# MarvelMathesh/sincformer-metacog-speech-enhancement

Measured on AMD Instinct MI355X. Metric: audio frames/sec/GPU (16 kHz, 512-frame utts) + mask RMSE vs CPU ref, higher is better.
Workload: dtype fp16 MFMA operands (PerceptionAgent, fusion, Conformer GEMMs, heads) + bf16 attention core, fp32 accumulate (ops.POLICIES['mixed']); 1 GPU; B256 x 512-frame utterances (L40880, T512) forward; batch_per_gpu=256, samples=40880, frames_per_utt=512, launch=eager launches, streams=3, precision_policy=mixed

## Files before the change

include/sincformer_hip.h:

```cpp
#ifndef SINCFORMER_HIP_H
#define SINCFORMER_HIP_H
#ifdef __cplusplus
extern "C" {
#endif

#define SFM_OK 0
#define SFM_ERR_ARG (-1)
#define SFM_ERR_SHAPE (-2)
#define SFM_ERR_LAUNCH (-3)
#define SFM_DT_BF16 0
#define SFM_DT_F16 1

#define SFM_EPI_NONE 0
#define SFM_EPI_SWISH 1
#define SFM_EPI_GELU 2
#define SFM_EPI_RESID 3
#define SFM_EPI_GLU 4
#define SFM_EPI_SIGMOID 5
#define SFM_EPI_TANH_SCALE 6
#define SFM_EPI_SIGMA 7
#define SFM_EPI_CPEA 8

int sfm_abi_version(void);

// ... 195 lines not shown
int sfm_layernorm_bwd_ex(const float* x, const float* gamma, const void* dy, int dy_16, const float* dres, float* dx,
                         float* dgamma, float* dbeta, int M, int D, int ldx, int ldy, int ld, float eps, int dtype,
                         float* ws, void* stream);
int sfm_layernorm_bwd_next(const float* x, const float* gamma, const void* dy, int dy_16, const float* dres, float* dx,
                           float* dgamma, float* dbeta, int M, int D, int ldx, int ldy, int ld, float eps, int dtype,
                           void* next16, float next_alpha, float next_p, unsigned int next_seed, float* ws, void* stream);
int sfm_ew_train(const void* z, const void* g, void* out, long long M, int N, int mode, int g_f32, int out_f32,
                 float alpha, float p, unsigned int seed, int dtype, void* stream);
long long sfm_col_stats_ws_floats(int M, int C);
int sfm_col_stats(const float* y, const float* aux, const float* mean, const float* rstd, float* S, int M, int C, float* ws,
                  void* stream);
int sfm_add_cols(const float* a, const float* b, float* out, long long M, int C, int Cb, long long lda, long long ldb, long long ldo,
                 void* stream);
int sfm_lstm_hprev16(const float* h, void* out, int B, int T, int H, int dtype, void* stream);
int sfm_bn_finalize(const float* S, const float* gamma, const float* beta, float* run_mean, float* run_var, float* mean,
                    float* rstd, float* sc, float* sh, int C, long long M, float eps, float momentum, int eval_mode,
                    void* stream);
int sfm_bn_swish_bwd(const void* g, const float* y, const float* mean, const float* rstd, const float* gamma,
                     const float* beta, float* S, float* dy, int M, int C, int g_f32, int pass, int dtype,
                     float* ws, void* stream);
long long sfm_dwconv_wgrad_scratch_floats(int B, int T, int C, int KS);
int sfm_dwconv_wgrad(const void* x, const float* dy, float* dw, float* db, float* scratch, int B, int T, int C, int KS,
                     int dtype, void* stream);
int sfm_attention_fwd_train(const void* qkv, void* out, float* lse, int B, int T, int H, int hd, int ldqkv,
                            int ldo, int koff, int voff, long long qkv_batch_stride, long long o_batch_stride,
                            float scale, float p_drop, unsigned int seed, int dtype, void* stream);
int sfm_attention_bwd(const void* qkv, const void* O, const void* dO, const float* lse, float* delta, void* dqkv,
                      int B, int T, int H, int hd, int ldqkv, int ldo, int koff, int voff, float p_drop,
                      unsigned int seed, int dtype, void* stream);
int sfm_lin256(const void* A, const void* W, const float* bias, void* out, int M, int NW, int lda, int ldo, int glu, int dtype,
               int out_dtype, void* stream);
int sfm_ln_lin256(const float* X32, int ldx, const float* lnw, const float* lnb, float eps, const void* W, const float* bias,
                  void* out, int M, int NW, int ldo, int glu, int dtype, int out_dtype, void* stream);
int sfm_headpool_frames_per_tile(int Tin, int Tout);
int sfm_headpool(const void* xd, const void* W, const float* bias, void* pooled, float* gn_partial, int B, int Tin, int Tout, int NW,
                 int lda, int ldp, int gcols, int dtype, void* stream);

int sfm_bilstm_layer(const float* xg, const float* whh, float* out, int B, int T, int H, int dtype, void* stream);
int sfm_bilstm_layer_ex(const float* xg, const float* whh, float* out, int B, int T, int H, int w16, void* stream);
int sfm_bilstm_layer_train_ex(const float* xg, const float* whh, float* out, float* save, int B, int T, int H, int w16, void* stream);
int sfm_bilstm_layer_train(const float* xg, const float* whh, float* out, float* save, int B, int T, int H, int dtype,
                           void* stream);
int sfm_bilstm_layer_bwd(const float* save, const float* whh, const float* dout, float* dxg, int B, int T, int H,
                         void* stream);
int sfm_memory_fwd(const float* emb, const float* params, float* bias_out, float* gate_out, int* top_idx,
                   float* sim_out, int B, int key_dim, int value_dim, int slots, float temperature, void* stream);
long long sfm_memory_param_floats(int key_dim, int value_dim, int slots);
int sfm_memory_bwd(const float* emb, const float* params, const float* d_out, const float* d_gate, float* d_emb,
                   float* dparams, int B, int key_dim, int value_dim, int slots, float temperature, float* ws, void* stream);

int sfm_pstoi_loss(const float* e0, const float* e1, const float* c0, const float* c1, const float* band_w, float* loss,
                   float* g0, float* g1, double* ws, int B, int T, int F, int NB, int frame_len, float beta_db, int layout,
                   void* stream);
int sfm_mse_loss(const float* pred, const float* target, float* loss, float* grad, double* ws, long long n, void* stream);

#ifdef __cplusplus
}
#endif
#endif
```

sincformer_metacog_speech_enhancement_amd/csrc/pointwise.hip:

```cpp
#include "sfm_common.h"

template <class T>
__global__ __launch_bounds__(256) void layernorm_kernel(const float* __restrict__ x, const float* __restrict__ w,
                                                        const float* __restrict__ bsh, u16* out16, float* out32,
                                                        int M, int D, int ldx, int ld16, int ld32, float eps, int act) {
  const int lane = threadIdx.x & 63;
  const int row = blockIdx.x * 4 + (threadIdx.x >> 6);
  if (row >= M) return;
  const float* xr = x + (long long)row * ldx;
  float v[8];
  float s = 0.f;
#pragma unroll
  for (int i = 0; i < 8; ++i) {
    int d = lane + 64 * i;
    v[i] = (d < D) ? xr[d] : 0.f;
    s += v[i];
  }
  const float mean = wave_sum(s) / (float)D;
  float q = 0.f;
#pragma unroll
  for (int i = 0; i < 8; ++i) {
    int d = lane + 64 * i;
    float c = (d < D) ? (v[i] - mean) : 0.f;
    q += c * c;
  }
  const float rstd = rsqrtf(wave_sum(q) / (float)D + eps);
#pragma unroll
  for (int i = 0; i < 8; ++i) {
    int d = lane + 64 * i;
    if (d < D) {
      float y = (v[i] - mean) * rstd * w[d] + bsh[d];
      if (act == 1) y = gelu_erf(y);
      if (out16) out16[(long long)row * ld16 + d] = T::from_f32(y);
// ... 993 lines not shown
  const long long total = M * F;
  for (long long e = (long long)blockIdx.x * 256 + threadIdx.x; e < total; e += (long long)gridDim.x * 256) {
    const long long m = e / F;
    const int f = (int)(e - m * F);
    const float r = re[e], i = im[e];
    const float gr = g[m * ld_g + f], gi = g[m * ld_g + F + f];
    const float mag = sqrtf(r * r + i * i + 1e-8f);
    const float nf = log1pf(mag) / mag;
    const float c = (gr * r + gi * i) * (1.0f / (1.0f + mag) - nf) / (mag * mag);
    dre[e] = gr * nf + c * r;
    dim_[e] = gi * nf + c * i;
  }
}

extern "C" int sfm_stft_lognorm_bwd(const float* re, const float* im, const float* g, float* dre, float* dim_, long long M, int F,
                                    long long ld_g, void* stream) {
  if (!re || !im || !g || !dre || !dim_) return SFM_ERR_ARG;
  if (M <= 0 || F <= 0 || ld_g < 2 * F) return SFM_ERR_SHAPE;
  long long nb = (M * F + 255) / 256;
  if (nb > 16384) nb = 16384;
  SFM_LAUNCH(stft_lognorm_bwd_kernel, dim3((unsigned)nb), dim3(256), 0, (hipStream_t)stream, re, im, g, dre, dim_, M, F, ld_g);
  return SFM_OK;
}

__global__ __launch_bounds__(256) void polar_mask_kernel(const float* __restrict__ lm, const float* __restrict__ lp,
                                                         const float* __restrict__ mag_bias, const float* __restrict__ nr,
                                                         const float* __restrict__ ni, float* mr, float* mi, float* er,
                                                         float* ei, float* mmag, long long rows_per_batch, int F,
                                                         long long total, float phase_scale, long long ld_l,
                                                         long long ld_enh) {
  for (long long e = (long long)blockIdx.x * 256 + threadIdx.x; e < total; e += (long long)gridDim.x * 256) {
    long long m = e / F;
    int f = (int)(e - m * F);
    float a = lm[m * ld_l + f];
    if (mag_bias) a += mag_bias[(m / rows_per_batch) * F + f];
    float mg = 1.0f / (1.0f + expf(-a));
    float ph = tanhf(lp[m * ld_l + f]) * phase_scale;
    float c = cosf(ph), s = sinf(ph);
    float xr = mg * c, xi = mg * s;
    if (mr) mr[e] = xr;
    if (mi) mi[e] = xi;
    if (mmag) mmag[e] = mg;
    if (er) {
      float r = nr[e], i = ni[e];
      er[m * ld_enh + f] = xr * r - xi * i;
      ei[m * ld_enh + f] = xr * i + xi * r;
    }
  }
}

extern "C" int sfm_polar_mask(const float* lm, const float* lp, const float* mag_bias, const float* nr, const float* ni,
                              float* mr, float* mi, float* er, float* ei, float* mmag, int B, long long rows_per_batch,
                              int F, float phase_scale, long long ld_logits, long long ld_enh, void* stream) {
  if (!lm || !lp) return SFM_ERR_ARG;
  if (er && (!ei || !nr || !ni)) return SFM_ERR_ARG;
  long long total = (long long)B * rows_per_batch * F;
  if (total <= 0) return SFM_ERR_SHAPE;
  long long nb = (total + 255) / 256;
  if (nb > 16384) nb = 16384;
  SFM_LAUNCH(polar_mask_kernel, dim3((unsigned)nb), dim3(256), 0, (hipStream_t)stream, lm, lp, mag_bias, nr, ni,
                     mr, mi, er, ei, mmag, rows_per_batch, F, total, phase_scale, ld_logits, ld_enh);
  return SFM_OK;
}

__global__ __launch_bounds__(256) void complex_mul_kernel(const float* __restrict__ sr, const float* __restrict__ si,
                                                          const float* __restrict__ mr, const float* __restrict__ mi,
                                                          float* er, float* ei, long long total) {
  for (long long e = (long long)blockIdx.x * 256 + threadIdx.x; e < total; e += (long long)gridDim.x * 256) {
    float a = sr[e], b = si[e], c = mr[e], d = mi[e];
    er[e] = c * a - d * b;
    ei[e] = c * b + d * a;
  }
}

extern "C" int sfm_complex_mul(const float* sr, const float* si, const float* mr, const float* mi, float* er, float* ei,
                               long long total, void* stream) {
  if (!sr || !si || !mr || !mi || !er || !ei) return SFM_ERR_ARG;
  if (total <= 0) return SFM_ERR_SHAPE;
  long long nb = (total + 255) / 256;
// ... 145 lines not shown
```

sincformer_metacog_speech_enhancement_amd/functional.py:

```python
import math
import numpy as np
import torch

from . import ops

N_FFT, HOP, WIN = 256, 80, 160
N_FREQ = N_FFT // 2 + 1
SINC_ON_16BIT_MFMA = True
FUSE_LD = 1088


def _f32(t):
    return t.detach().float().contiguous()


def sub(sd, prefix):
    p = prefix + "."
    return {k[len(p):]: v for k, v in sd.items() if k.startswith(p)}


def add_to16(x32, y32, C):
    M = x32.numel() // C
    dev = x32.device
    one = _const(dev, C, 1.0)
# ... 350 lines not shown
    with ops.stage("block", pk.get("index")):
        return _block_forward(x32, pk, B, T, H, want16, seg)


def _block_forward(x32, pk, B, T, H, want16, seg=None):
    if _ffn_fusable(x32, pk["ff1"]) and x32.shape[1] == 256:
        x, h = ffn_forward_ln(x32, pk["ff1"], pk["mhsa"]["ln_w"], pk["mhsa"]["ln_b"], False, True)
        x = mhsa_forward(x, pk["mhsa"], B, T, H, h=h, index=pk.get("index"), seg=seg)
        x = convmod_forward(x, pk["conv"], B, T, seg=seg)
        if not want16 and _ffn_fusable(x, pk["ff2"]):
            return ffn_forward_ln(x, pk["ff2"], pk["fn_w"], pk["fn_b"], True, False)[1]
        x = ffn_forward(x, pk["ff2"])
    else:
        x = ffn_forward(x32, pk["ff1"])
        x = mhsa_forward(x, pk["mhsa"], B, T, H, index=pk.get("index"), seg=seg)
        x = convmod_forward(x, pk["conv"], B, T, seg=seg)
        x = ffn_forward(x, pk["ff2"])
    out = torch.empty_like(x)
    out16 = torch.empty(x.shape, device=x.device, dtype=ops.compute_dtype()) if want16 else None
    ops.layernorm(x, pk["fn_w"], pk["fn_b"], out16=out16, out32=out)
    return (out, out16) if want16 else out


def pack_complex_conformer(sd, num_blocks, num_heads=4):
    nf2 = sd["input_proj.weight"].shape[1]
    with ops.stage("front"):
        win = ops.pack_linear(sd["input_proj.weight"], sd["input_proj.bias"], k_pad_to=ops.round_up(nf2, 64))
    with ops.stage("tail"):
        wout = ops.pack_linear(sd["output_proj.weight"], sd["output_proj.bias"])
    return {"in": win, "out": wout,
            "blocks": [pack_block(sub(sd, "blocks.%d" % i), num_heads, i) for i in range(num_blocks)], "nf2": nf2}


def complex_conformer_core(x16, pk, B, T, H, out_dtype=None):
    with ops.stage("front"):
        x = ops.linear16(x16, pk["in"], out_dtype=torch.float32)
    skip = x
    for bp in pk["blocks"]:
        x = block_forward(x, bp, B, T, H)
    with ops.stage("tail"):
        y16 = add_to16(x, skip, x.shape[1])
        return ops.linear16(y16, pk["out"], out_dtype=out_dtype or ops.compute_dtype())


def complex_conformer_forward(stft_real, stft_imag, pk, H):
    B, T, nf = stft_real.shape
    M = B * T
    sr, si = stft_real.contiguous(), stft_imag.contiguous()
    ld = pk["in"].Kpad
    with ops.stage("front"):
        x16 = torch.empty(M, ld, device=sr.device, dtype=ops.compute_dtype())
        ops.convert_rows(sr, x16, M, nf, nf, nf, ld)
        ops.convert_rows(si, x16[:, nf:], M, nf, ld - nf, nf, ld)
    y = complex_conformer_core(x16, pk, B, T, H, out_dtype=torch.float32).reshape(B, T, 2 * nf)
    return y[..., :nf], y[..., nf:]


def pack_perception(sd, sample_rate):
    with ops.stage("pa"):
        return _pack_perception(sd, sample_rate)


def _pack_perception(sd, sample_rate):
    pk = {"fs": float(sample_rate)}
    for k in ("low_hz_", "band_hz_", "window", "n_"):
        pk[k] = _f32(sd["sinc_conv." + k]).reshape(-1)
    pk["K"] = pk["window"].numel()
    pk["C0"] = pk["low_hz_"].numel()
    pk["sn_w"], pk["sn_b"] = _f32(sd["sinc_norm.weight"]), _f32(sd["sinc_norm.bias"])
    pk["blocks"] = []
    for i in range(3):
        s = sub(sd, "conv_blocks.%d" % i)
# ... 187 lines not shown
        h = ops.bilstm_layer(xg, lp["whh"], B, T, H, w16=ops.lstm_w16())
        x16 = torch.empty(M, 2 * H, device=h.device, dtype=dt)
        ops.convert_rows(h, x16, M, 2 * H, 2 * H, 2 * H, 2 * H)
    oc = pk["oc"]
    if out is None:
        out = torch.empty(M, 4 * oc, device=x16.device, dtype=torch.float32)
    ops.linear16(x16, pk["heads"], epi=ops.EPI_CPEA, alpha=math.pi, nsplit=2 * oc, out=out)
    return out


def pack_memory_params(sd):
    order = ["key_proj.0.weight", "key_proj.0.bias", "key_proj.1.weight", "key_proj.1.bias", "key_proj.3.weight",
             "key_proj.3.bias", "keys", "values", "value_proj.0.weight", "value_proj.0.bias", "gate.0.weight",
             "gate.0.bias"]
    return torch.cat([_f32(sd[k]).reshape(-1) for k in order]).contiguous()


def pack_msa(sd, num_blocks, num_heads=4):
    with ops.stage("front"):
        pk = {"f0": ops.pack_linear(sd["fusion.0.weight"], sd["fusion.0.bias"], k_pad_to=FUSE_LD),
              "f1w": _f32(sd["fusion.1.weight"]), "f1b": _f32(sd["fusion.1.bias"]),
              "f3": ops.pack_linear(sd["fusion.3.weight"], sd["fusion.3.bias"]),
              "f4w": _f32(sd["fusion.4.weight"]), "f4b": _f32(sd["fusion.4.bias"])}
    pk["conf"] = pack_complex_conformer(sub(sd, "conformer"), num_blocks, num_heads)
    with ops.stage("tail"):
        pk.update({"r0": ops.pack_linear(sd["mask_proj_real.0.weight"], sd["mask_proj_real.0.bias"]),
                   "r2": ops.pack_linear(sd["mask_proj_real.2.weight"], sd["mask_proj_real.2.bias"]),
                   "i0": ops.pack_linear(sd["mask_proj_imag.0.weight"], sd["mask_proj_imag.0.bias"]),
                   "i2": ops.pack_linear(sd["mask_proj_imag.2.weight"], sd["mask_proj_imag.2.bias"])})
    pk["d_model"] = sd["fusion.3.weight"].shape[0]
    return pk


def msa_logits(fused16, pk, B, T, H):
    D = pk["d_model"]
    with ops.stage("front"):
        h = ops.linear16(fused16, pk["f0"], out_dtype=torch.float32)
        h16 = _ln16(h, pk["f1w"], pk["f1b"], act=1)
        h = ops.linear16(h16, pk["f3"], out_dtype=torch.float32)
        hf16 = _ln16(h, pk["f4w"], pk["f4b"])
    y16 = complex_conformer_core(hf16, pk["conf"], B, T, H)
    half = D // 2
    with ops.stage("tail"):
        gr = ops.linear16(y16[:, :half], pk["r0"], epi=ops.EPI_GELU)
        lm = ops.linear16(gr, pk["r2"], out_dtype=torch.float32)
        gi = ops.linear16(y16[:, half:], pk["i0"], epi=ops.EPI_GELU)
        lp = ops.linear16(gi, pk["i2"], out_dtype=torch.float32)
    return lm, lp


def msa_pack_inputs(z_real, z_imag, cpea, noisy_real, noisy_imag):
    with ops.stage("front"):
        return _msa_pack_inputs(z_real, z_imag, cpea, noisy_real, noisy_imag)


def _msa_pack_inputs(z_real, z_imag, cpea, noisy_real, noisy_imag):
    B, D, T = z_real.shape
    M = B * T
    dev = z_real.device
    fused = torch.empty(M, FUSE_LD, device=dev, dtype=ops.compute_dtype())
    zr, zi = z_real.float().contiguous(), z_imag.float().contiguous()
    ops.transpose(zr, fused, B, D, T, D * T, T, T * FUSE_LD, FUSE_LD)
    ops.transpose(zi, fused[:, D:], B, D, T, D * T, T, T * FUSE_LD, FUSE_LD)
    col = 2 * D
    for k in ("rho_s", "rho_n", "phi1", "phi2"):
        c = cpea[k].float().contiguous()
        oc = c.shape[-1]
        ops.convert_rows(c, fused[:, col:], M, oc, oc, oc, FUSE_LD)
        col += oc
    nr, ni = noisy_real.float().contiguous(), noisy_imag.float().contiguous()
    F = nr.shape[-1]
    ops.stft_lognorm_pack(nr, ni, fused[:, col:], M, F, FUSE_LD - col - 2 * F, FUSE_LD)
    return fused, nr, ni


PHASE_SCALE_MSA = 3.14159 / 8.0


def msa_forward(z_real, z_imag, cpea, noisy_real, noisy_imag, pk, H, mag_bias=None):
    B, D, T = z_real.shape
    fused, nr, ni = msa_pack_inputs(z_real, z_imag, cpea, noisy_real, noisy_imag)
    lm, lp = msa_logits(fused, pk, B, T, H)
    F = nr.shape[-1]
    mr = torch.empty(B, T, F, device=lm.device, dtype=torch.float32)
    mi = torch.empty(B, T, F, device=lm.device, dtype=torch.float32)
    ops.polar_mask(lm, lp, B, T, F, PHASE_SCALE_MSA, lm.stride(0), mag_bias=mag_bias, mr=mr, mi=mi)
    return mr, mi


def enhance_path(wave, packs, H=4, use_memory=False, want=("mask", "wave")):
    dt = ops.stage_dtype("front")
    wave = wave.contiguous()
    B, L = wave.shape
    dev = wave.device
    T = 1 + L // HOP
    M = B * T
    pa = packs["pa"]
    D = pa["D"]
    want_lat = "latents" in want
    zcat, sigma = perception_forward(wave, pa, latents=want_lat, pool_to=T)
    zsrc, zsc, zsh = (zcat, None, None) if want_lat else zcat
    Tpa = zsrc.shape[1]
    fused = torch.empty(M, FUSE_LD, device=dev, dtype=dt)
    with ops.stage("front"):
        ops.pool_time(zsrc, fused, None, B, Tpa, T, 2 * D, 2 * D, FUSE_LD, scale=zsc, shift=zsh)
    oc4 = 4 * packs["cpea"]["oc"]
    cpea_forward(fused, packs["cpea"], B, T, out=fused[:, 2 * D:2 * D + oc4])
    nr, ni = (stft_split16 if FUSED_STFT_SPLIT16 else stft)(wave)
    col = 2 * D + oc4
    with ops.stage("front"):
        ops.stft_lognorm_pack(nr, ni, fused[:, col:], M, N_FREQ, FUSE_LD - col - 2 * N_FREQ, FUSE_LD)
    bias = None
    out = {}
    if use_memory:
        params, kd, vd, slots, temp = packs["memory"]
        zpool = torch.empty(B, T, kd, device=dev, dtype=torch.float32)
        ops.pool_time(zsrc, None, zpool, B, Tpa, T, kd, 2 * D, kd, scale=zsc[:, :kd].contiguous(), shift=zsh[:, :kd].contiguous())
        emb_r = ops.mean_time(zpool, B, T, kd, kd)
        bias, gate, top, sim = ops.memory_fwd(emb_r, params, kd, vd, slots, temp)
        out.update(mem_bias=bias, mem_gate=gate, mem_top=top, mem_sim=sim)
    lm, lp = msa_logits(fused, packs["msa"], B, T, H)
    mr = torch.empty(B, T, N_FREQ, device=dev, dtype=torch.float32)
    mi = torch.empty(B, T, N_FREQ, device=dev, dtype=torch.float32)
    ld = ops.round_up(2 * N_FREQ, 8)
    spec = torch.zeros(M, ld, device=dev, dtype=torch.float32)
    ops.polar_mask(lm, lp, B, T, N_FREQ, PHASE_SCALE_MSA, lm.stride(0), mag_bias=bias, nr=nr, ni=ni, mr=mr, mi=mi,
                   er=spec, ei=spec[:, N_FREQ:], ld_enh=ld)
    out.update(mask_real=mr, mask_imag=mi, sigma=sigma, noisy_real=nr, noisy_imag=ni, spec=spec)
    if want_lat:
        out["zcat"] = zcat
    if "wave" in want:
        out["enhanced"] = (istft_from_packed_split16 if FUSED_STFT_SPLIT16 else istft_from_packed)(spec, B, T, L)
    return out


MR_STFT = ((256, 64, 256), (512, 128, 512), (1024, 256, 1024))



_COUNTS = {}


def counts_tensor(counts, device):
    key = (counts, str(device))
    t = _COUNTS.get(key)
    if t is None:
        t = _COUNTS[key] = torch.tensor(list(counts), device=device, dtype=torch.int64)
    return t


def enhancer_loss(enh_real, enh_imag, clean_wave, clean_real, clean_imag):
    B, L = clean_wave.shape
    enh_wav = istft(enh_real, enh_imag, L)
    Sw = ops.wave_moments(enh_wav, clean_wave.contiguous())
    Sm = ops.spec_sums(enh_real.contiguous(), enh_imag.contiguous(), clean_real.contiguous(), clean_imag.contiguous())
    Sr = torch.zeros(len(MR_STFT), 4, device=clean_wave.device, dtype=torch.float64)
    counts = []
    for i, (nf, hp, wn) in enumerate(MR_STFT):
        pr, pi = stft(enh_wav, nf, hp, wn)
        tr, ti = stft(clean_wave, nf, hp, wn)
# ... 6 lines not shown
```

sincformer_metacog_speech_enhancement_amd/lib.py:

```python
import ctypes
import os

import torch

_HERE = os.path.dirname(os.path.abspath(__file__))
LIB_PATH = os.environ.get("SFM_LIB_PATH") or os.path.join(_HERE, "libsincformer_hip.so")

c_vp = ctypes.c_void_p
c_i = ctypes.c_int
c_ll = ctypes.c_longlong
c_f = ctypes.c_float

SIGNATURES = {
    "sfm_abi_version": [],
    "sfm_gemm16": [c_vp, c_vp, c_vp, c_vp, c_vp, c_vp, c_i, c_i, c_i, c_i, c_i, c_i, c_i, c_i, c_ll, c_i, c_i, c_i,
                   c_i, c_ll, c_i, c_ll, c_f, c_i, c_i, c_i, c_i, c_i, c_vp],
    "sfm_gemm16_ex": [c_vp, c_vp, c_vp, c_vp, c_vp, c_vp, c_i, c_i, c_i, c_i, c_i, c_i, c_i, c_i, c_ll, c_i, c_i, c_i,
                   c_i, c_ll, c_i, c_ll, c_f, c_i, c_i, c_i, c_i, c_i, c_i, c_vp],
    "sfm_gemm16_train": [c_vp, c_vp, c_vp, c_vp, c_vp, c_vp, c_i, c_i, c_i, c_i, c_i, c_i, c_i, c_i, c_ll, c_i, c_i, c_i,
                   c_i, c_ll, c_i, c_ll, c_f, c_i, c_i, c_i, c_i, c_i, c_i, c_f, ctypes.c_uint, c_vp],
    "sfm_conv16p": [c_vp, c_vp, c_vp, c_vp, c_vp, c_vp, c_vp, c_vp, c_vp, c_vp, c_vp, c_vp, c_vp, c_vp, c_i, c_i, c_i, c_i, c_i,
                    c_i, c_i, c_i, c_i, c_i, c_vp],
    "sfm_framed_gemm_f32": [c_vp, c_vp, c_vp, c_vp, c_vp, c_vp, c_i, c_i, c_i, c_ll, c_i, c_i, c_i, c_i, c_i, c_i,
                            c_i, c_ll, c_ll, c_ll, c_i, c_i, c_i, c_i, c_vp],
# ... 64 lines not shown
    "sfm_sumsq": [c_vp, c_ll, c_vp, c_vp, c_vp],
    "sfm_adamw_step": [c_vp, c_vp, c_vp, c_vp, c_ll, c_vp, c_f, c_f, c_f, c_f, c_f, c_f, c_f, c_i, c_vp],
    "sfm_adamw_step_masked": [c_vp, c_vp, c_vp, c_vp, c_ll, c_vp, c_f, c_f, c_f, c_f, c_f, c_f, c_f, c_i, c_vp, c_vp, c_i, c_vp],
    "sfm_adamw_step_scaled": [c_vp, c_vp, c_vp, c_vp, c_ll, c_vp, c_f, c_f, c_f, c_f, c_f, c_f, c_f, c_i, c_vp, c_vp, c_i, c_vp,
                              c_f, c_f, c_i, c_vp],
    "sfm_tn_ws_floats": [c_i, c_i, c_i],
    "sfm_colsum_ws_floats": [c_i, c_i],
    "sfm_layernorm_bwd_ws_floats": [c_i, c_i],
    "sfm_col_stats_ws_floats": [c_i, c_i],
    "sfm_gn_bwd_reduce_ws_floats": [c_i, c_i, c_i],
    "sfm_gemm16_tn": [c_vp, c_vp, c_vp, c_vp, c_i, c_i, c_i, c_i, c_i, c_i, c_i, c_vp, c_ll, c_vp],
    "sfm_conv_wgrad16": [c_vp, c_vp, c_vp, c_vp, c_i, c_i, c_i, c_i, c_i, c_i, c_i, c_i, c_ll, c_i, c_i, c_i, c_vp, c_ll, c_vp],
    "sfm_colsum": [c_vp, c_vp, c_i, c_i, c_i, c_i, c_i, c_vp, c_vp],
    "sfm_layernorm_bwd": [c_vp, c_vp, c_vp, c_vp, c_vp, c_vp, c_vp, c_i, c_i, c_i, c_i, c_f, c_vp, c_vp],
    "sfm_layernorm_bwd_ex": [c_vp, c_vp, c_vp, c_i, c_vp, c_vp, c_vp, c_vp, c_i, c_i, c_i, c_i, c_i, c_f, c_i, c_vp, c_vp],
    "sfm_layernorm_bwd_next": [c_vp, c_vp, c_vp, c_i, c_vp, c_vp, c_vp, c_vp, c_i, c_i, c_i, c_i, c_i, c_f, c_i, c_vp, c_f, c_f,
                               ctypes.c_uint, c_vp, c_vp],
    "sfm_ew_train": [c_vp, c_vp, c_vp, c_ll, c_i, c_i, c_i, c_i, c_f, c_f, ctypes.c_uint, c_i, c_vp],
    "sfm_col_stats": [c_vp, c_vp, c_vp, c_vp, c_vp, c_i, c_i, c_vp, c_vp],
    "sfm_add_cols": [c_vp, c_vp, c_vp, c_ll, c_i, c_i, c_ll, c_ll, c_ll, c_vp],
    "sfm_lstm_hprev16": [c_vp, c_vp, c_i, c_i, c_i, c_i, c_vp],
    "sfm_bn_finalize": [c_vp, c_vp, c_vp, c_vp, c_vp, c_vp, c_vp, c_vp, c_vp, c_i, c_ll, c_f, c_f, c_i, c_vp],
    "sfm_bn_swish_bwd": [c_vp, c_vp, c_vp, c_vp, c_vp, c_vp, c_vp, c_vp, c_i, c_i, c_i, c_i, c_i, c_vp, c_vp],
    "sfm_dwconv_wgrad": [c_vp, c_vp, c_vp, c_vp, c_vp, c_i, c_i, c_i, c_i, c_i, c_vp],
    "sfm_dwconv_wgrad_scratch_floats": [c_i, c_i, c_i, c_i],
    "sfm_attention_fwd_train": [c_vp, c_vp, c_vp, c_i, c_i, c_i, c_i, c_i, c_i, c_i, c_i, c_ll, c_ll, c_f, c_f,
                                ctypes.c_uint, c_i, c_vp],
    "sfm_attention_bwd": [c_vp, c_vp, c_vp, c_vp, c_vp, c_vp, c_i, c_i, c_i, c_i, c_i, c_i, c_i, c_i, c_f,
                          ctypes.c_uint, c_i, c_vp],
    "sfm_lin256": [c_vp, c_vp, c_vp, c_vp, c_i, c_i, c_i, c_i, c_i, c_i, c_i, c_vp],
    "sfm_headpool_frames_per_tile": [c_i, c_i],
    "sfm_headpool": [c_vp, c_vp, c_vp, c_vp, c_vp, c_i, c_i, c_i, c_i, c_i, c_i, c_i, c_i, c_vp],
    "sfm_ln_lin256": [c_vp, c_i, c_vp, c_vp, c_f, c_vp, c_vp, c_vp, c_i, c_i, c_i, c_i, c_i, c_i, c_vp],
    "sfm_bilstm_layer": [c_vp, c_vp, c_vp, c_i, c_i, c_i, c_i, c_vp],
    "sfm_bilstm_layer_ex": [c_vp, c_vp, c_vp, c_i, c_i, c_i, c_i, c_vp],
    "sfm_bilstm_layer_train": [c_vp, c_vp, c_vp, c_vp, c_i, c_i, c_i, c_i, c_vp],
    "sfm_bilstm_layer_train_ex": [c_vp, c_vp, c_vp, c_vp, c_i, c_i, c_i, c_i, c_vp],
    "sfm_bilstm_layer_bwd": [c_vp, c_vp, c_vp, c_vp, c_i, c_i, c_i, c_vp],
    "sfm_memory_fwd": [c_vp, c_vp, c_vp, c_vp, c_vp, c_vp, c_i, c_i, c_i, c_i, c_f, c_vp],
    "sfm_memory_bwd": [c_vp, c_vp, c_vp, c_vp, c_vp, c_vp, c_i, c_i, c_i, c_i, c_f, c_vp, c_vp],
    "sfm_memory_param_floats": [c_i, c_i, c_i],
    "sfm_framed_gemm_f32_varlen": [c_vp, c_vp, c_vp, c_vp, c_vp, c_vp, c_i, c_i, c_i, c_i, c_i, c_i, c_i, c_i, c_i, c_ll, c_ll,
                                   c_i, c_i, c_i, c_vp],
    "sfm_framed_gemm_split16_varlen": [c_vp, c_vp, c_vp, c_vp, c_vp, c_vp, c_vp, c_i, c_i, c_i, c_i, c_i, c_i, c_i, c_i, c_i, c_i,
                                       c_ll, c_i, c_vp],
    "sfm_attention_fwd_varlen": [c_vp, c_vp, c_vp, c_vp, c_i, c_i, c_i, c_i, c_i, c_i, c_i, c_i, c_i, c_i, c_f, c_i, c_i, c_vp],
    "sfm_dwconv_folded_varlen": [c_vp, c_vp, c_vp, c_vp, c_vp, c_vp, c_vp, c_i, c_i, c_i, c_i, c_i, c_i, c_i, c_i, c_i, c_vp],
    "sfm_istft_ola_varlen": [c_vp, c_vp, c_vp, c_vp, c_vp, c_i, c_i, c_i, c_i, c_i, c_ll, c_vp],
    "sfm_pstoi_loss": [c_vp, c_vp, c_vp, c_vp, c_vp, c_vp, c_vp, c_vp, c_vp, c_i, c_i, c_i, c_i, c_i, c_f, c_i, c_vp],
    "sfm_mse_loss": [c_vp, c_vp, c_vp, c_vp, c_vp, c_ll, c_vp],
}

RETURNS_LONG_LONG = {
    "sfm_mean_time_scratch_floats", "sfm_sinc_wgrad_scratch_floats", "sfm_sinc_shift_len", "sfm_gn_bwd_reduce_ws_floats",
    "sfm_tn_ws_floats", "sfm_colsum_ws_floats", "sfm_layernorm_bwd_ws_floats", "sfm_col_stats_ws_floats",
    "sfm_dwconv_wgrad_scratch_floats", "sfm_memory_param_floats",
}

_lib = None


class HipExtensionMissing(RuntimeError):
    pass


def load():
# ... 26 lines not shown
```

sincformer_metacog_speech_enhancement_amd/ops.py:

```python
import ctypes
import math
import numpy as np
import torch

from . import lib as _lib

EPI_NONE, EPI_SWISH, EPI_GELU, EPI_RESID, EPI_GLU, EPI_SIGMOID, EPI_TANH_SCALE, EPI_SIGMA, EPI_CPEA = range(9)

_DT_ID = {torch.bfloat16: 0, torch.float16: 1}
import os as _os
TRAIN_DTYPE = torch.float16
_state = {"dtype": TRAIN_DTYPE}

_SWITCHES = {
    "gemm_variant": ["SFM_GEMM_VARIANT", 0, 0],
    "attention_variant": [None, 0, 0],
    "lin256": ["SFM_LIN256", True, True],
    "headpool": ["SFM_HEADPOOL", True, True],
    "lstm_w16": ["SFM_LSTM_W16", True, True],
    "deterministic": ["SFM_DETERMINISTIC", True, True],
    "wgrad_stream": ["SFM_WGRAD_STREAM", True, True],
    "fuse_ffn_swish": ["SFM_FUSE_FFN_SWISH", True, True],
    "fuse_next_drop": ["SFM_FUSE_NEXT_DROP", True, True],
    "steal_grads": ["SFM_STEAL_GRADS", False, False],
    "lstm_bwd_lpu": ["SFM_LSTM_BWD_LPU", 4, 4],
}
for _sw in _SWITCHES.values():
    if _sw[0] is not None and _sw[0] in _os.environ:
        _sw[2] = (_os.environ[_sw[0]] != "0") if isinstance(_sw[1], bool) else int(_os.environ[_sw[0]])


def switch(name):
    return _SWITCHES[name][2]


def variant_overrides():
    return {name: cur for name, (_, default, cur) in _SWITCHES.items() if cur != default}


def set_gemm_variant(v):
    _SWITCHES["gemm_variant"][2] = int(v)


_DT_NAMES = {"bf16": torch.bfloat16, "bfloat16": torch.bfloat16, "f16": torch.float16, "fp16": torch.float16,
             "float16": torch.float16}
STAGES = ("pa", "front", "block", "attn", "tail")
POLICIES = {
    "bf16": {s: torch.bfloat16 for s in STAGES},
    "fp16": {s: torch.float16 for s in STAGES},
    "mixed": {"pa": torch.float16, "front": torch.float16, "block": torch.float16, "attn": torch.bfloat16,
              "tail": torch.float16},
# ... 611 lines not shown
    dsrc = torch.empty(B, Tin, C, device=dout32.device, dtype=torch.float32)
    _call("pool_time_bwd", L.sfm_pool_time_bwd, (_p(dout32), _p(dsrc), B, Tin, Tout, C, C, C, _stream()), 0.0,
          4.0 * B * (Tin + Tout) * C)
    return dsrc


def pool_time(src32, dst16, dst32, B, Tin, Tout, C, ld_src, ld_dst, scale=None, shift=None):
    L = _lib.load()
    src_bytes = src32.element_size()
    if src_bytes == 4:
        args = (_p(src32), _p(scale), _p(shift), _p(dst16), _p(dst32), B, Tin, Tout, C, ld_src, ld_dst, _dt(), _stream())
        fn = L.sfm_pool_time_affine
    else:
        args = (_p(src32), _DT_ID[src32.dtype], _p(scale), _p(shift), _p(dst16), _p(dst32), B, Tin, Tout, C, ld_src, ld_dst,
                _dt(), _stream())
        fn = L.sfm_pool_time_affine16
    _call("pool_time", fn, args, *_cost_of("pool_time", locals()))


def stft_lognorm_pack(re, im, dst16, M, F, zpad, ld_dst):
    L = _lib.load()
    _call("stft_lognorm_pack", L.sfm_stft_lognorm_pack, (_p(re), _p(im), _p(dst16), M, F, zpad, ld_dst, _dt(), _stream()),
          *_cost_of("stft_lognorm_pack", locals()))


def polar_mask(lm, lp, B, rows, F, phase_scale, ld_logits, mag_bias=None, nr=None, ni=None, mr=None, mi=None, er=None,
               ei=None, mmag=None, ld_enh=0):
    L = _lib.load()
    _call("polar_mask", L.sfm_polar_mask, (_p(lm), _p(lp), _p(mag_bias), _p(nr), _p(ni), _p(mr), _p(mi), _p(er), _p(ei), _p(mmag), B,
                          rows, F, float(phase_scale), ld_logits, ld_enh, _stream()),
          *_cost_of("polar_mask", locals()))


def complex_mul(sr, si, mr, mi):
    L = _lib.load()
    er, ei = torch.empty_like(sr), torch.empty_like(sr)
    _call("complex_mul", L.sfm_complex_mul, (_p(sr), _p(si), _p(mr), _p(mi), _p(er), _p(ei), sr.numel(), _stream()),
          *_cost_of("complex_mul", locals()))
    return er, ei


def istft_ola(frames, win2, out, B, T, Ln, n_fft, hop, win, ld_frames):
    L = _lib.load()
    _call("istft_ola", L.sfm_istft_ola, (_p(frames), _p(win2), _p(out), B, T, Ln, n_fft, hop, win, ld_frames, _stream()),
          *_cost_of("istft_ola", locals()))


ATTN_QTILE = 128
DWCONV_TILE = 64
_XCDS, _XCD_RUN = 8, 8


def attention_items(frame_counts, H):
    T = np.asarray(frame_counts, dtype=np.int64)
    order = np.argsort(-T, kind="stable")
    nt = (T[order] + ATTN_QTILE - 1) // ATTN_QTILE
    per = np.repeat(nt, H)
    n = int(per.sum())
    utt = np.repeat(np.repeat(order, H), per)
    head = np.repeat(np.tile(np.arange(H), len(T)), per)
    first = np.repeat(np.cumsum(per) - per, per)
    tile = np.arange(n) - first
    logical = np.stack([utt, head, tile, np.zeros(n, dtype=np.int64)], axis=1)
    run = _XCDS * _XCD_RUN
    pos = np.arange(n)
    base = pos // run * run
# ... 781 lines not shown
```

Before: 8.581 million STFT frames/s (whole job).

## Fuse MSA mask tail: residual add, out proj, heads, polar mask into one kernel

Adds a single HIP kernel that runs the whole MSA tail for a 128-row tile. It does the residual add, the 256x256 output projection, both GELU head layers, both logit projections, the polar mask and the enhanced-spectrum write, keeping activations in LDS and staging weights through double-buffered buffer-to-LDS loads. This removes about six separate GEMM and pointwise launches and their fp16 and fp32 intermediate round trips through HBM. It uses about 137 KB of LDS and 512 threads per block, which limits occupancy, and it falls back to the old path when shapes or packing do not match.

```diff
diff --git a/include/sincformer_hip.h b/include/sincformer_hip.h
--- a/include/sincformer_hip.h
+++ b/include/sincformer_hip.h
@@ -251,6 +251,10 @@
                int out_dtype, void* stream);
 int sfm_ln_lin256(const float* X32, int ldx, const float* lnw, const float* lnb, float eps, const void* W, const float* bias,
                   void* out, int M, int NW, int ldo, int glu, int dtype, int out_dtype, void* stream);
+int sfm_mask_tail(const float* x, const float* skip, const void* w_out, const float* b_out, const void* w_r0, const float* b_r0,
+                  const void* w_i0, const float* b_i0, const void* w_r2, const float* b_r2, const void* w_i2, const float* b_i2,
+                  const float* mag_bias, const float* nr, const float* ni, float* mr, float* mi, float* spec, int M,
+                  int rows_per_batch, int ld_spec, float phase_scale, int dtype, void* stream);
 int sfm_headpool_frames_per_tile(int Tin, int Tout);
 int sfm_headpool(const void* xd, const void* W, const float* bias, void* pooled, float* gn_partial, int B, int Tin, int Tout, int NW,
                  int lda, int ldp, int gcols, int dtype, void* stream);
diff --git a/sincformer_metacog_speech_enhancement_amd/csrc/mask_tail.hip b/sincformer_metacog_speech_enhancement_amd/csrc/mask_tail.hip
--- /dev/null
+++ b/sincformer_metacog_speech_enhancement_amd/csrc/mask_tail.hip
@@ -0,0 +1,318 @@
+#include "sfm_common.h"
+#include "polar_epi.h"
+
+#define MT_BM 128
+#define MT_F 129
+#define MT_CHUNK 32768
+#define MT_OFF_W 65536
+#define MT_IMG (MT_BM * MT_F)
+#define MT_OFF_BIAS (2 * MT_IMG * 4)
+#define MT_NBIAS 896
+#define MT_LDS (MT_OFF_BIAS + MT_NBIAS * 4 + MT_BM * 4)
+
+struct MtParams {
+  const float* x;
+  const float* skip;
+  const u16 *w_out, *w_r0, *w_i0, *w_r2, *w_i2;
+  const float *b_out, *b_r0, *b_i0, *b_r2, *b_i2;
+  const float* mag_bias;
+  const float *nr, *ni;
+  float *mr, *mi;
+  float* spec;
+  int M, rows_per_batch, ld;
+  float phase_scale;
+};
+
+template <class T>
+__global__ __launch_bounds__(512) void mask_tail_kernel(MtParams p) {
+  extern __shared__ __attribute__((aligned(16))) unsigned char smem[];
+  unsigned char* act = smem;
+  unsigned char* wb0 = smem + MT_OFF_W;
+  unsigned char* wb1 = wb0 + MT_CHUNK;
+  float* bs = reinterpret_cast<float*>(smem + MT_OFF_BIAS);
+  int* rowb = reinterpret_cast<int*>(bs + MT_NBIAS);
+
+  const int tid = threadIdx.x, lane = tid & 63;
+  const int wave = __builtin_amdgcn_readfirstlane(tid >> 6);
+  const int l31 = lane & 31, hl = lane >> 5;
+  const int half = wave & 1;
+  const int r1 = (wave >> 1) * 32 + l31;
+  const int m0 = blockIdx.x * MT_BM;
+  const int M = p.M;
+  auto rs_out = __builtin_amdgcn_make_buffer_rsrc((void*)p.w_out, 0, 256 * 256 * 2, 0x00020000);
+  auto rs_r0 = __builtin_amdgcn_make_buffer_rsrc((void*)p.w_r0, 0, 128 * 128 * 2, 0x00020000);
+  auto rs_i0 = __builtin_amdgcn_make_buffer_rsrc((void*)p.w_i0, 0, 128 * 128 * 2, 0x00020000);
+  auto rs_r2 = __builtin_amdgcn_make_buffer_rsrc((void*)p.w_r2, 0, 192 * 128 * 2, 0x00020000);
+  auto rs_i2 = __builtin_amdgcn_make_buffer_rsrc((void*)p.w_i2, 0, 192 * 128 * 2, 0x00020000);
+
+  auto load_wout = [&](int c, unsigned char* dst) {
+#pragma unroll
+    for (int i = 0; i < 4; ++i) {
+      const int inst = wave * 4 + i;
+      const int row = inst * 2 + (lane >> 5);
+      const int lc = (lane & 31) ^ (row & 15);
+      __builtin_amdgcn_raw_ptr_buffer_load_lds(rs_out, (lds_ptr_t)(dst + inst * 1024), 16, ((c * 64 + row) * 256 + lc * 8) * 2, 0, 0, 0);
+    }
+  };
+  auto load_k128 = [&](decltype(rs_r0) rs, int row0, unsigned char* dst, int inst0, int n) {
+#pragma unroll
+    for (int i = 0; i < 4; ++i) {
+      if (i < n) {
+        const int inst = inst0 + i;
+        const int row = inst * 4 + (lane >> 4);
+        const int lc = (lane & 15) ^ (row & 15);
+        __builtin_amdgcn_raw_ptr_buffer_load_lds(rs, (lds_ptr_t)(dst + inst * 1024), 16, ((row0 + row) * 128 + lc * 8) * 2, 0, 0, 0);
+      }
+    }
+  };
+  auto load_head0 = [&](int im, unsigned char* dst) {
+    if (im) load_k128(rs_i0, 0, dst, wave * 4, 4);
+    else load_k128(rs_r0, 0, dst, wave * 4, 4);
+  };
+  auto load_head2 = [&](int j, unsigned char* dst) {
+    if (wave < 4) load_k128(rs_r2, j * 64, dst, wave * 4, 4);
+    else load_k128(rs_i2, j * 64, dst + 16384, (wave - 4) * 4, 4);
+  };
+  auto wfrag = [&](const unsigned char* base, int n, int pitch, int k) {
+    return *reinterpret_cast<const u32x4*>(base + n * pitch + (((2 * k + hl) ^ (n & 15)) << 4));
+  };
+
+  load_wout(0, wb0);
+  load_wout(1, wb1);
+  for (int i = tid; i < MT_NBIAS; i += 512) {
+    float v;
+    if (i < 256) v = p.b_out[i];
+    else if (i < 384) v = p.b_r0[i - 256];
+    else if (i < 512) v = p.b_i0[i - 384];
+    else if (i < 704) v = p.b_r2[i - 512];
+    else v = p.b_i2[i - 704];
+    bs[i] = v;
+  }
+  if (tid < MT_BM) {
+    const int m = min(m0 + tid, M - 1);
+    rowb[tid] = (m / p.rows_per_batch) * MT_F;
+  }
+
+  {
+    f32x4 xv[16], sv[16];
+#pragma unroll
+    for (int r = 0; r < 16; ++r) {
+      const int m = min(m0 + wave * 16 + r, M - 1);
+      xv[r] = *reinterpret_cast<const f32x4*>(p.x + (long long)m * 256 + 4 * lane);
+      sv[r] = *reinterpret_cast<const f32x4*>(p.skip + (long long)m * 256 + 4 * lane);
+    }
+#pragma unroll
+    for (int r = 0; r < 16; ++r) {
+      const int row = wave * 16 + r;
+      float y[4];
+#pragma unroll
+      for (int j = 0; j < 4; ++j) y[j] = fmaf(sv[r][j], 1.0f, fmaf(xv[r][j], 1.0f, 0.0f));
+      u32x2 pk;
+      pk[0] = pack2<T>(y[0], y[1]);
+      pk[1] = pack2<T>(y[2], y[3]);
+      *reinterpret_cast<u32x2*>(act + row * 512 + (((lane >> 1) ^ (row & 15)) << 4) + (lane & 1) * 8) = pk;
+    }
+  }
+  wait_vmcnt<0>();
+  ring_barrier();
+  u32x4 hf[16];
+#pragma unroll
+  for (int s = 0; s < 16; ++s) hf[s] = *reinterpret_cast<const u32x4*>(act + r1 * 512 + (((2 * s + hl) ^ (r1 & 15)) << 4));
+  ring_barrier();
+
+  auto put16 = [&](const f32x16& s, const float* bias, int col0, bool gelu) {
+#pragma unroll
+    for (int q = 0; q < 4; ++q) {
+      const int n = 8 * q + 4 * hl;
+      const f32x4 bv = *reinterpret_cast<const f32x4*>(bias + n);
+      float y[4];
+#pragma unroll
+      for (int e = 0; e < 4; ++e) {
+        y[e] = s[4 * q + e] + bv[e];
+        if (gelu) y[e] = gelu_erf(y[e]);
+      }
+      u32x2 pk;
+      pk[0] = pack2<T>(y[0], y[1]);
+      pk[1] = pack2<T>(y[2], y[3]);
+      const int col = col0 + n;
+      *reinterpret_cast<u32x2*>(act + r1 * 512 + (((col >> 3) ^ (r1 & 15)) << 4) + hl * 8) = pk;
+    }
+  };
+
+#pragma unroll
+  for (int c = 0; c < 4; ++c) {
+    unsigned char* wb = (c & 1) ? wb1 : wb0;
+    if (c >= 2) {
+      wait_vmcnt<4>();
+      ring_barrier();
+    }
+    f32x16 s;
+#pragma unroll
+    for (int r = 0; r < 16; ++r) s[r] = 0.f;
+    const int n1 = half * 32 + l31;
+#pragma unroll
+    for (int k = 0; k < 16; ++k) s = T::mfma(wfrag(wb, n1, 512, k), hf[k], s);
+    put16(s, bs + c * 64 + half * 32, c * 64 + half * 32, false);
+    ring_barrier();
+    if (c < 2) load_wout(c + 2, wb);
+    else load_head0(c - 2, wb);
+  }
+
+  wait_vmcnt<0>();
+  ring_barrier();
+  {
+    u32x4 yf[8];
+#pragma unroll
+    for (int s = 0; s < 8; ++s) yf[s] = *reinterpret_cast<const u32x4*>(act + r1 * 512 + (((half * 16 + 2 * s + hl) ^ (r1 & 15)) << 4));
+    const unsigned char* wb = half ? wb1 : wb0;
+#pragma unroll
+    for (int j = 0; j < 4; ++j) {
+      f32x16 s;
+#pragma unroll
+      for (int r = 0; r < 16; ++r) s[r] = 0.f;
+#pragma unroll
+      for (int k = 0; k < 8; ++k) s = T::mfma(wfrag(wb, 32 * j + l31, 256, k), yf[k], s);
+      put16(s, bs + 256 + half * 128 + 32 * j, half * 128 + 32 * j, true);
+    }
+  }
+  ring_barrier();
+  load_head2(0, wb0);
+  load_head2(1, wb1);
+
+  u32x4 gf[16];
+#pragma unroll
+  for (int s = 0; s < 16; ++s) gf[s] = *reinterpret_cast<const u32x4*>(act + r1 * 512 + (((2 * s + hl) ^ (r1 & 15)) << 4));
+  auto head2 = [&](const unsigned char* wb, int lt, f32x16& lm, f32x16& lp) {
+#pragma unroll
+    for (int r = 0; r < 16; ++r) lm[r] = lp[r] = 0.f;
+    const int n1 = lt * 32 + l31;
+#pragma unroll
+    for (int k = 0; k < 8; ++k) lm = T::mfma(wfrag(wb, n1, 256, k), gf[k], lm);
+#pragma unroll
+    for (int k = 0; k < 8; ++k) lp = T::mfma(wfrag(wb + 16384, n1, 256, k), gf[8 + k], lp);
+  };
+  f32x16 lm0, lp0, lm1, lp1;
+  float lm4 = 0.f, lp4 = 0.f;
+  wait_vmcnt<4>();
+  ring_barrier();
+  head2(wb0, half, lm0, lp0);
+  ring_barrier();
+  load_head2(2, wb0);
+  wait_vmcnt<4>();
+  ring_barrier();
+  head2(wb1, half, lm1, lp1);
+  wait_vmcnt<0>();
+  ring_barrier();
+  if (half == 0) {
+    f32x16 a, b;
+    head2(wb0, 0, a, b);
+    lm4 = a[0];
+    lp4 = b[0];
+  }
+  ring_barrier();
+
+  float* LM = reinterpret_cast<float*>(smem);
+  float* LP = LM + MT_IMG;
+  auto put32 = [&](const f32x16& lm, const f32x16& lp, int t) {
+#pragma unroll
+    for (int q = 0; q < 4; ++q)
+#pragma unroll
+      for (int e = 0; e < 4; ++e) {
+        const int n = 32 * t + 8 * q + 4 * hl + e;
+        LM[r1 * MT_F + n] = lm[4 * q + e] + bs[512 + n];
+        LP[r1 * MT_F + n] = lp[4 * q + e] + bs[704 + n];
+      }
+  };
+  put32(lm0, lp0, half);
+  put32(lm1, lp1, 2 + half);
+  if (half == 0 && hl == 0) {
+    LM[r1 * MT_F + 128] = lm4 + bs[512 + 128];
+    LP[r1 * MT_F + 128] = lp4 + bs[704 + 128];
+  }
+  ring_barrier();
+
+  const long long e0 = (long long)m0 * MT_F, total = (long long)M * MT_F;
+  const bool enh = p.spec != nullptr;
+#pragma unroll 1
+  for (int u = tid; u < MT_IMG / 4; u += 512) {
+    const int el = u * 4;
+    const long long e = e0 + el;
+    if (e >= total) break;
+    const bool full = e + 4 <= total;
+    const f32x4 a4 = *reinterpret_cast<const f32x4*>(LM + el), p4 = *reinterpret_cast<const f32x4*>(LP + el);
+    f32x4 r4 = {0.f, 0.f, 0.f, 0.f}, i4 = {0.f, 0.f, 0.f, 0.f};
+    if (enh) {
+      if (full) {
+        r4 = *reinterpret_cast<const f32x4*>(p.nr + e);
+        i4 = *reinterpret_cast<const f32x4*>(p.ni + e);
+      } else {
+#pragma unroll
+        for (int j = 0; j < 4; ++j)
+          if (e + j < total) { r4[j] = p.nr[e + j]; i4[j] = p.ni[e + j]; }
+      }
+    }
+    int row = el / MT_F, f = el - row * MT_F;
+    f32x4 xr4, xi4, er4, ei4;
+#pragma unroll
+    for (int j = 0; j < 4; ++j) {
+      float xr, xi, mg, er, ei;
+      sfm_polar_unit(a4[j], p.mag_bias ? p.mag_bias + rowb[row] + f : nullptr, p4[j], p.phase_scale, xr, xi, mg);
+      sfm_polar_apply(xr, xi, r4[j], i4[j], er, ei);
+      xr4[j] = xr; xi4[j] = xi; er4[j] = er; ei4[j] = ei;
+      if (++f == MT_F) {
+        f = 0;
+        row = min(row + 1, MT_BM - 1);
+      }
+    }
+    if (full) {
+      *reinterpret_cast<f32x4*>(p.mr + e) = xr4;
+      *reinterpret_cast<f32x4*>(p.mi + e) = xi4;
+    } else {
+#pragma unroll
+      for (int j = 0; j < 4; ++j)
+        if (e + j < total) { p.mr[e + j] = xr4[j]; p.mi[e + j] = xi4[j]; }
+    }
+    *reinterpret_cast<f32x4*>(LM + el) = er4;
+    *reinterpret_cast<f32x4*>(LP + el) = ei4;
+  }
+  if (!enh) return;
+  ring_barrier();
+
+  const int upr = p.ld >> 2;
+#pragma unroll 1
+  for (int u = tid; u < MT_BM * upr; u += 512) {
+    const int row = u / upr, c0 = (u - row * upr) * 4;
+    if (m0 + row >= M) break;
+    f32x4 v;
+#pragma unroll
+    for (int j = 0; j < 4; ++j) {
+      const int c = c0 + j;
+      v[j] = c < MT_F ? LM[row * MT_F + c] : (c < 2 * MT_F ? LP[row * MT_F + c - MT_F] : 0.f);
+    }
+    *reinterpret_cast<f32x4*>(p.spec + (long long)(m0 + row) * p.ld + c0) = v;
+  }
+}
+
+extern "C" int sfm_mask_tail(const float* x, const float* skip, const void* w_out, const float* b_out, const void* w_r0,
+                             const float* b_r0, const void* w_i0, const float* b_i0, const void* w_r2, const float* b_r2,
+                             const void* w_i2, const float* b_i2, const float* mag_bias, const float* nr, const float* ni, float* mr,
+                             float* mi, float* spec, int M, int rows_per_batch, int ld_spec, float phase_scale, int dtype,
+                             void* stream) {
+  if (!x || !skip || !w_out || !b_out || !w_r0 || !b_r0 || !w_i0 || !b_i0 || !w_r2 || !b_r2 || !w_i2 || !b_i2 || !mr || !mi)
+    return SFM_ERR_ARG;
+  if (spec && (!nr || !ni)) return SFM_ERR_ARG;
+  if (dtype != SFM_DT_BF16 && dtype != SFM_DT_F16) return SFM_ERR_ARG;
+  if (M <= 0 || M > (1 << 30) || rows_per_batch <= 0) return SFM_ERR_SHAPE;
+  if (spec && (ld_spec < 2 * MT_F || (ld_spec % 4) != 0 || ld_spec > 4096)) return SFM_ERR_SHAPE;
+  if ((((uintptr_t)x | (uintptr_t)skip | (uintptr_t)nr | (uintptr_t)ni | (uintptr_t)mr | (uintptr_t)mi | (uintptr_t)spec |
+        (uintptr_t)w_out | (uintptr_t)w_r0 | (uintptr_t)w_i0 | (uintptr_t)w_r2 | (uintptr_t)w_i2) % 16) != 0)
+    return SFM_ERR_SHAPE;
+  MtParams p = {x, skip, (const u16*)w_out, (const u16*)w_r0, (const u16*)w_i0, (const u16*)w_r2, (const u16*)w_i2,
+                b_out, b_r0, b_i0, b_r2, b_i2, mag_bias, spec ? nr : nullptr, spec ? ni : nullptr, mr, mi, spec,
+                M, rows_per_batch, ld_spec, phase_scale};
+  dim3 grid((M + MT_BM - 1) / MT_BM), block(512);
+  hipStream_t st = (hipStream_t)stream;
+  if (dtype == SFM_DT_F16) SFM_LAUNCH_LDS((mask_tail_kernel<F16>), grid, block, MT_LDS, st, p);
+  else SFM_LAUNCH_LDS((mask_tail_kernel<BF16>), grid, block, MT_LDS, st, p);
+  return SFM_OK;
+}
diff --git a/sincformer_metacog_speech_enhancement_amd/csrc/pointwise.hip b/sincformer_metacog_speech_enhancement_amd/csrc/pointwise.hip
--- a/sincformer_metacog_speech_enhancement_amd/csrc/pointwise.hip
+++ b/sincformer_metacog_speech_enhancement_amd/csrc/pointwise.hip
@@ -1,4 +1,5 @@
 #include "sfm_common.h"
+#include "polar_epi.h"
 
 template <class T>
 __global__ __launch_bounds__(256) void layernorm_kernel(const float* __restrict__ x, const float* __restrict__ w,
@@ -1058,19 +1059,17 @@
   for (long long e = (long long)blockIdx.x * 256 + threadIdx.x; e < total; e += (long long)gridDim.x * 256) {
     long long m = e / F;
     int f = (int)(e - m * F);
-    float a = lm[m * ld_l + f];
-    if (mag_bias) a += mag_bias[(m / rows_per_batch) * F + f];
-    float mg = 1.0f / (1.0f + expf(-a));
-    float ph = tanhf(lp[m * ld_l + f]) * phase_scale;
-    float c = cosf(ph), s = sinf(ph);
-    float xr = mg * c, xi = mg * s;
+    float xr, xi, mg;
+    sfm_polar_unit(lm[m * ld_l + f], mag_bias ? mag_bias + (m / rows_per_batch) * F + f : nullptr, lp[m * ld_l + f], phase_scale,
+                   xr, xi, mg);
     if (mr) mr[e] = xr;
     if (mi) mi[e] = xi;
     if (mmag) mmag[e] = mg;
     if (er) {
-      float r = nr[e], i = ni[e];
-      er[m * ld_enh + f] = xr * r - xi * i;
-      ei[m * ld_enh + f] = xr * i + xi * r;
+      float vr, vi;
+      sfm_polar_apply(xr, xi, nr[e], ni[e], vr, vi);
+      er[m * ld_enh + f] = vr;
+      ei[m * ld_enh + f] = vi;
     }
   }
 }
diff --git a/sincformer_metacog_speech_enhancement_amd/csrc/polar_epi.h b/sincformer_metacog_speech_enhancement_amd/csrc/polar_epi.h
--- /dev/null
+++ b/sincformer_metacog_speech_enhancement_amd/csrc/polar_epi.h
@@ -0,0 +1,18 @@
+#pragma once
+#include "sfm_common.h"
+
+__device__ __forceinline__ void sfm_polar_unit(float a, const float* __restrict__ bias, float lp, float phase_scale, float& xr,
+                                               float& xi, float& mg) {
+  if (bias) a += *bias;
+  mg = 1.0f / (1.0f + expf(-a));
+  float ph = tanhf(lp) * phase_scale;
+  float c = cosf(ph), s = sinf(ph);
+  xr = mg * c;
+  xi = mg * s;
+}
+
+__device__ __forceinline__ void sfm_polar_apply(float xr, float xi, float r, float i, float& er, float& ei) {
+#pragma clang fp contract(off)
+  er = xr * r - xi * i;
+  ei = xr * i + xi * r;
+}
diff --git a/sincformer_metacog_speech_enhancement_amd/functional.py b/sincformer_metacog_speech_enhancement_amd/functional.py
--- a/sincformer_metacog_speech_enhancement_amd/functional.py
+++ b/sincformer_metacog_speech_enhancement_amd/functional.py
@@ -406,12 +406,17 @@
             "blocks": [pack_block(sub(sd, "blocks.%d" % i), num_heads, i) for i in range(num_blocks)], "nf2": nf2}
 
 
-def complex_conformer_core(x16, pk, B, T, H, out_dtype=None):
+def complex_conformer_stream(x16, pk, B, T, H):
     with ops.stage("front"):
         x = ops.linear16(x16, pk["in"], out_dtype=torch.float32)
     skip = x
     for bp in pk["blocks"]:
         x = block_forward(x, bp, B, T, H)
+    return x, skip
+
+
+def complex_conformer_core(x16, pk, B, T, H, out_dtype=None):
+    x, skip = complex_conformer_stream(x16, pk, B, T, H)
     with ops.stage("tail"):
         y16 = add_to16(x, skip, x.shape[1])
         return ops.linear16(y16, pk["out"], out_dtype=out_dtype or ops.compute_dtype())
@@ -665,21 +670,55 @@
     return pk
 
 
-def msa_logits(fused16, pk, B, T, H):
-    D = pk["d_model"]
+def _msa_fusion(fused16, pk):
     with ops.stage("front"):
         h = ops.linear16(fused16, pk["f0"], out_dtype=torch.float32)
         h16 = _ln16(h, pk["f1w"], pk["f1b"], act=1)
         h = ops.linear16(h16, pk["f3"], out_dtype=torch.float32)
-        hf16 = _ln16(h, pk["f4w"], pk["f4b"])
-    y16 = complex_conformer_core(hf16, pk["conf"], B, T, H)
-    half = D // 2
+        return _ln16(h, pk["f4w"], pk["f4b"])
+
+
+def _msa_heads(y16, pk):
+    half = pk["d_model"] // 2
     with ops.stage("tail"):
         gr = ops.linear16(y16[:, :half], pk["r0"], epi=ops.EPI_GELU)
         lm = ops.linear16(gr, pk["r2"], out_dtype=torch.float32)
         gi = ops.linear16(y16[:, half:], pk["i0"], epi=ops.EPI_GELU)
         lp = ops.linear16(gi, pk["i2"], out_dtype=torch.float32)
     return lm, lp
+
+
+def msa_logits(fused16, pk, B, T, H):
+    y16 = complex_conformer_core(_msa_fusion(fused16, pk), pk["conf"], B, T, H)
+    return _msa_heads(y16, pk)
+
+
+def msa_tail(x, skip, pk, B, T, mag_bias=None, nr=None, ni=None):
+    F = pk["r2"].N
+    M, dev = B * T, x.device
+    mr = torch.empty(B, T, F, device=dev, dtype=torch.float32)
+    mi = torch.empty(B, T, F, device=dev, dtype=torch.float32)
+    ld = ops.round_up(2 * F, 8)
+    with ops.stage("tail"):
+        tail = (pk["conf"]["out"], pk["r0"], pk["i0"], pk["r2"], pk["i2"])
+        if ops.mask_tail_ok(x, skip, *tail, F):
+            spec = torch.empty(M, ld, device=dev, dtype=torch.float32) if nr is not None else None
+            ops.mask_tail(x, skip, *tail, T, PHASE_SCALE_MSA, mr, mi, mag_bias=mag_bias, nr=nr, ni=ni, spec=spec)
+            return mr, mi, spec
+        y16 = ops.linear16(add_to16(x, skip, x.shape[1]), pk["conf"]["out"])
+    lm, lp = _msa_heads(y16, pk)
+    if nr is None:
+        ops.polar_mask(lm, lp, B, T, F, PHASE_SCALE_MSA, lm.stride(0), mag_bias=mag_bias, mr=mr, mi=mi)
+        return mr, mi, None
+    spec = torch.zeros(M, ld, device=dev, dtype=torch.float32)
+    ops.polar_mask(lm, lp, B, T, F, PHASE_SCALE_MSA, lm.stride(0), mag_bias=mag_bias, nr=nr, ni=ni, mr=mr, mi=mi,
+                   er=spec, ei=spec[:, F:], ld_enh=ld)
+    return mr, mi, spec
+
+
+def msa_masks(fused16, pk, B, T, H, mag_bias=None, nr=None, ni=None):
+    x, skip = complex_conformer_stream(_msa_fusion(fused16, pk), pk["conf"], B, T, H)
+    return msa_tail(x, skip, pk, B, T, mag_bias=mag_bias, nr=nr, ni=ni)
 
 
 def msa_pack_inputs(z_real, z_imag, cpea, noisy_real, noisy_imag):
@@ -713,11 +752,7 @@
 def msa_forward(z_real, z_imag, cpea, noisy_real, noisy_imag, pk, H, mag_bias=None):
     B, D, T = z_real.shape
     fused, nr, ni = msa_pack_inputs(z_real, z_imag, cpea, noisy_real, noisy_imag)
-    lm, lp = msa_logits(fused, pk, B, T, H)
-    F = nr.shape[-1]
-    mr = torch.empty(B, T, F, device=lm.device, dtype=torch.float32)
-    mi = torch.empty(B, T, F, device=lm.device, dtype=torch.float32)
-    ops.polar_mask(lm, lp, B, T, F, PHASE_SCALE_MSA, lm.stride(0), mag_bias=mag_bias, mr=mr, mi=mi)
+    mr, mi, _ = msa_masks(fused, pk, B, T, H, mag_bias=mag_bias)
     return mr, mi
 
 
@@ -752,13 +787,7 @@
         emb_r = ops.mean_time(zpool, B, T, kd, kd)
         bias, gate, top, sim = ops.memory_fwd(emb_r, params, kd, vd, slots, temp)
         out.update(mem_bias=bias, mem_gate=gate, mem_top=top, mem_sim=sim)
-    lm, lp = msa_logits(fused, packs["msa"], B, T, H)
-    mr = torch.empty(B, T, N_FREQ, device=dev, dtype=torch.float32)
-    mi = torch.empty(B, T, N_FREQ, device=dev, dtype=torch.float32)
-    ld = ops.round_up(2 * N_FREQ, 8)
-    spec = torch.zeros(M, ld, device=dev, dtype=torch.float32)
-    ops.polar_mask(lm, lp, B, T, N_FREQ, PHASE_SCALE_MSA, lm.stride(0), mag_bias=bias, nr=nr, ni=ni, mr=mr, mi=mi,
-                   er=spec, ei=spec[:, N_FREQ:], ld_enh=ld)
+    mr, mi, spec = msa_masks(fused, packs["msa"], B, T, H, mag_bias=bias, nr=nr, ni=ni)
     out.update(mask_real=mr, mask_imag=mi, sigma=sigma, noisy_real=nr, noisy_imag=ni, spec=spec)
     if want_lat:
         out["zcat"] = zcat
diff --git a/sincformer_metacog_speech_enhancement_amd/lib.py b/sincformer_metacog_speech_enhancement_amd/lib.py
--- a/sincformer_metacog_speech_enhancement_amd/lib.py
+++ b/sincformer_metacog_speech_enhancement_amd/lib.py
@@ -120,6 +120,7 @@
     "sfm_headpool_frames_per_tile": [c_i, c_i],
     "sfm_headpool": [c_vp, c_vp, c_vp, c_vp, c_vp, c_i, c_i, c_i, c_i, c_i, c_i, c_i, c_i, c_vp],
     "sfm_ln_lin256": [c_vp, c_i, c_vp, c_vp, c_f, c_vp, c_vp, c_vp, c_i, c_i, c_i, c_i, c_i, c_i, c_vp],
+    "sfm_mask_tail": [c_vp] * 18 + [c_i, c_i, c_i, c_f, c_i, c_vp],
     "sfm_bilstm_layer": [c_vp, c_vp, c_vp, c_i, c_i, c_i, c_i, c_vp],
     "sfm_bilstm_layer_ex": [c_vp, c_vp, c_vp, c_i, c_i, c_i, c_i, c_vp],
     "sfm_bilstm_layer_train": [c_vp, c_vp, c_vp, c_vp, c_i, c_i, c_i, c_i, c_vp],
diff --git a/sincformer_metacog_speech_enhancement_amd/ops.py b/sincformer_metacog_speech_enhancement_amd/ops.py
--- a/sincformer_metacog_speech_enhancement_amd/ops.py
+++ b/sincformer_metacog_speech_enhancement_amd/ops.py
@@ -17,6 +17,7 @@
     "attention_variant": [None, 0, 0],
     "lin256": ["SFM_LIN256", True, True],
     "headpool": ["SFM_HEADPOOL", True, True],
+    "mask_tail": [None, True, True],
     "lstm_w16": ["SFM_LSTM_W16", True, True],
     "deterministic": ["SFM_DETERMINISTIC", True, True],
     "wgrad_stream": ["SFM_WGRAD_STREAM", True, True],
@@ -694,6 +695,49 @@
           *_cost_of("polar_mask", locals()))
 
 
+def set_mask_tail(flag):
+    _SWITCHES["mask_tail"][2] = bool(flag)
+
+
+MASK_TAIL_F = 129
+
+
+def mask_tail_ok(x32, skip32, wout, r0, i0, r2, i2, F):
+    dt = _state["dtype"]
+
+    def packed(pw, n, npad, k):
+        return (pw.N == n and pw.K == k and pw.Npad == npad and pw.Kpad == k and pw.ksize == 1 and not pw.glu and
+                pw.w.dtype == dt and pw.w.is_contiguous() and pw.bias is not None and pw.bias.numel() == npad)
+
+    return (switch("mask_tail") and switch("gemm_variant") == 0 and dt in _DT_ID and F == MASK_TAIL_F and
+            x32.dim() == 2 and x32.shape[1] == 256 and x32.dtype == torch.float32 and skip32.dtype == torch.float32 and
+            x32.shape == skip32.shape and x32.is_contiguous() and skip32.is_contiguous() and
+            packed(wout, 256, 256, 256) and packed(r0, 128, 128, 128) and packed(i0, 128, 128, 128) and
+            packed(r2, F, 192, 128) and packed(i2, F, 192, 128))
+
+
+def mask_tail(x32, skip32, wout, r0, i0, r2, i2, rows_per_batch, phase_scale, mr, mi, mag_bias=None, nr=None, ni=None, spec=None):
+    _need_dev(x32, skip32, mr, mi)
+    L = _lib.load()
+    M = x32.shape[0]
+    F = MASK_TAIL_F
+    for t in (mr, mi, nr, ni, spec, mag_bias):
+        if t is not None and (t.dtype != torch.float32 or not t.is_contiguous()):
+            raise RuntimeError("mask_tail: fp32 contiguous operands only")
+    if mr.numel() != M * F or mi.numel() != M * F or (spec is not None and (nr is None or ni is None or spec.shape[0] != M)):
+        raise RuntimeError("mask_tail: operand shapes do not match M = %d" % M)
+    wbytes = 2.0 * (256 * 256 + 2 * 128 * 128 + 2 * 192 * 128)
+    flops = 2.0 * M * (256 * 256 + 2 * 128 * 128 + 2 * 128 * F) + 20.0 * M * F
+    nbytes = M * (2 * 256 * 4.0 + 2 * F * 4.0) + wbytes
+    if spec is not None:
+        nbytes += M * (2 * F * 4.0 + spec.shape[1] * 4.0)
+    _call("mask_tail", L.sfm_mask_tail, (_p(x32), _p(skip32), _p(wout.w), _p(wout.bias), _p(r0.w), _p(r0.bias), _p(i0.w), _p(i0.bias),
+                                         _p(r2.w), _p(r2.bias), _p(i2.w), _p(i2.bias), _p(mag_bias), _p(nr), _p(ni), _p(mr), _p(mi),
+                                         _p(spec), M, int(rows_per_batch), spec.shape[1] if spec is not None else 0,
+                                         float(phase_scale), _dt(), _stream()),
+          flops, nbytes, tag="M%d%s" % (M, " +spec" if spec is not None else ""))
+
+
 def complex_mul(sr, si, mr, mi):
     L = _lib.load()
     er, ei = torch.empty_like(sr), torch.empty_like(sr)
```

New measurement: 8.650 million STFT frames/s (whole job), median of 4. About the same (+0.8%).
